# ohjay/snn-modulation-classification

Hardware: AMD Instinct MI355X
Metric: IQ windows/sec (RadioML 2x128, T=128) (higher is better)
Workload: dtype f32

## Files before the change

include/dcll_hip.h:

```cpp
#ifndef DCLL_HIP_H
#define DCLL_HIP_H

#include <stdint.h>

#ifdef __cplusplus
extern "C" {
#endif

#define DCLL_ABI_VERSION 10

enum {
    DCLL_OK = 0,
    DCLL_ERR_INVALID = -1,
    DCLL_ERR_UNSUPPORTED = -2,
    DCLL_ERR_LAUNCH = -3
};

typedef struct dcll_conv_desc {
    int32_t c_in, c_out;
    int32_t h, w;
    int32_t kh, kw;
    int32_t pad_h, pad_w;
    int32_t stride, dilation, groups;
    int32_t pool_h, pool_w;
// ... 336 lines not shown
#define DCLL_BWD_ANY     1
#define DCLL_BWD_WIDE    2
#define DCLL_BWD_SLAB    3
#define DCLL_BWD_BANDS   4
#define DCLL_BWD_POOL_DV 1u
int dcll_conv_lif_backward_ex(const dcll_conv_desc *d, const float *eps1, const float *v, const float *pv_pooled,
                              const float *g_p, const float *g_o, const float *g_pv, const float *g_v, const float *i2o_W,
                              float *dW, float *db, float *d_outW, float *d_outb, float *scratch, int64_t scratch_floats,
                              int32_t B, int32_t path, int32_t bands, uint32_t flags, void *stream);
int dcll_conv_lif_backward_ex_open(const dcll_conv_desc *d, const float *eps1, const float *v, const float *pv_pooled,
                                   const float *g_p, const float *g_o, const float *g_pv, const float *g_v, const float *i2o_W,
                                   float *d_outW, float *d_outb, float *scratch, int64_t scratch_floats, int32_t B,
                                   const float **part, int32_t *nchunk, int32_t path, int32_t bands, uint32_t flags, void *stream);
int32_t dcll_bwd_dv_pool_served(const dcll_conv_desc *d, int32_t B);

#ifdef __cplusplus
}
#endif
#endif
```

snn_modulation_classification_amd/_lib.py:

```python
import ctypes
import os
import subprocess

_PKG = os.path.dirname(os.path.abspath(__file__))
SO_PATH = os.environ.get("DCLL_HIP_SO") or os.path.join(_PKG, "libdcll_hip.so")
CSRC = os.path.join(_PKG, "csrc")

DCLL_OK, DCLL_ERR_INVALID, DCLL_ERR_UNSUPPORTED, DCLL_ERR_LAUNCH = 0, -1, -2, -3
ABI_VERSION = 10


class DCLLHipError(RuntimeError):
    pass


class DCLLUnsupported(NotImplementedError):
    pass


class ConvDesc(ctypes.Structure):
    _fields_ = [(n, ctypes.c_int32) for n in
                ("c_in", "c_out", "h", "w", "kh", "kw", "pad_h", "pad_w", "stride", "dilation", "groups",
                 "pool_h", "pool_w", "target", "output_layer", "tau_is_tensor", "refractory")] + \
               [("alpharp", ctypes.c_float), ("wrp", ctypes.c_float)]
# ... 87 lines not shown
    "dcll_grad_reduce_optim": (_I32, [ctypes.POINTER(GradParts), _I32, ctypes.POINTER(OptimTensor), _I32, _P, _P]),
    "dcll_conv_lif_backward_open_multi": (_I32, [ctypes.POINTER(BwdItem), _I32, _P]),
    "dcll_cells_to_planes": (_I32, [_P, _P, _I64, _I32, _P]),
    "dcll_dense_lif_step": (_I32, [_DDP] + [_P] * 16 + [_I32, _P]),
    "dcll_dense_lif_sequence": (_I32, [_DDP] + [_P] * 16 + [_I32, _I32, _P]),
    "dcll_dense_lif_backward": (_I32, [_DDP] + [_P] * 9 + [_I64, _I32, _P]),
    "dcll_dense_lif_backward_open": (_I32, [_DDP] + [_P] * 7 + [_I64, _I32, ctypes.POINTER(ctypes.c_void_p), _IP, _P]),
    "dcll_conv_lif_sequence": (_I32, [_DP] + [_P] * 13 + [_I32, _P, _P, _I32, _OP, _I32, _I32, _P]),
    "dcll_permute_readout": (_I32, [_P, _P, _I32, _P]),
    "dcll_conv_lif_sequence_cells": (_I32, [_DP] + [_P] * 10 + [_P, _P, _I32, _OP, _I32, _I32, _P]),
    "dcll_conv_lif_sequence_iq": (_I32, [_DP, _P, _P, _P, _P, _I32, _I32] + [_P] * 9 + [_P, _P, _I32, _OP, _I32, _I32, _P]),
    "dcll_pv_lowhigh": (_I32, [_P, _I64, _I32, _I32, _P, _P]),
    "dcll_pv_lowhigh_act": (_I32, [_P, _I64, _I32, _I32, _P, _I32, _P]),
    "dcll_readout_act_scratch": (_I64, [_I64, _I32, _I32]),
    "dcll_readout_act": (_I32, [_P] * 5 + [_I64, _I64, _I32, _I32, _I32, _P]),
    "dcll_pv_lowhigh_steps": (_I32, [_I32, _I32]),
    "dcll_readout": (_I32, [_P, _P, _P, _P, _I64, _I32, _I32, _P]),
    "dcll_readout_mode": (_I32, [_P, _P, _P, _P, _I64, _I32, _I32, _I32, _P]),
    "dcll_readout_splitk_scratch": (_I64, [_I64, _I32, _I32]),
    "dcll_readout_splitk": (_I32, [_P, _P, _P, _P, _P, _I64, _I64, _I32, _I32, _P]),
    "dcll_vote_tallies": (_I32, [_P, _I32, _P, _P, _I32, _I32, _P]),
    "dcll_step_readouts_scratch": (_I64, [_I64, _I32, _I32, _I32]),
    "dcll_step_readouts": (_I32, [_P, _P, _P, _P, _I64, _I64, _I32, _I32, _I32, _P, _P, _P, _P, _P, _P, _I32, _P]),
    "dcll_step_readouts_multi": (_I32, [ctypes.POINTER(StepRo), _I32, _P]),
    "dcll_argmax_vote": (_I32, [_P, _P, _P, _I32, _I32, _I32, _I32, _P]),
    "dcll_iq_encode": (_I32, [_P, _P, _P, _P, _P, _I32, _I32, _I32, _I32, _I32, _I32, _P]),
    "dcll_unpack_spikes": (_I32, [_P, _P, _I64, _P]),
    "dcll_pack_spikes": (_I32, [_P, _P, _I64, _P]),
    "dcll_conv_lif_sequence_any_lds": (_I64, [_DP]),
    "dcll_conv_lif_sequence_any_scratch": (_I64, [_DP]),
# ... 117 lines not shown
```

snn_modulation_classification_amd/csrc/dcll_hip.hip:

```cpp
#include "dcll_internal.h"
#include <map>
#include <mutex>
#include <utility>

static thread_local char g_err[DCLL_ERR_LEN] = "";
char *dcll_err_buf(void) { return g_err; }

extern "C" int dcll_version(void) { return DCLL_ABI_VERSION; }
extern "C" const char *dcll_last_error(void) { return g_err; }

constexpr size_t DCLL_TRACE_LEN = 1 << 16;
static thread_local bool g_trace_on = false;
static thread_local size_t g_trace_len = 0;
static thread_local char *g_trace = nullptr;
void dcll_trace_note(const char *name)
{
    if (!g_trace_on || !g_trace) return;
    const size_t n = strlen(name);
    if (g_trace_len + n + 5 >= DCLL_TRACE_LEN) {
        if (g_trace_len + 4 < DCLL_TRACE_LEN && (g_trace_len < 4 || memcmp(g_trace + g_trace_len - 4, "...\n", 4) != 0)) {
            memcpy(g_trace + g_trace_len, "...\n", 4);
            g_trace_len += 4;
        }
        return;
// ... 1883 lines not shown
                constexpr int ROW = decltype(ROWC)::value;
                const auto prs0 = tile_rsrc(pv_out + ubase), prs1 = tile_rsrc(pv_out + ubase + ustep);
                const auto vrs0 = tile_rsrc(v_out + ubase), vrs1 = tile_rsrc(v_out + ubase + ustep);
                uint32_t pk = 0;
#pragma unroll
                for (int m = 0; m < 8; ++m) {
                    const auto sw = __builtin_amdgcn_permlane16_swap(__float_as_uint(acc[2 * m]), __float_as_uint(acc[2 * m + 1]), false, false);
                    float v0 = __uint_as_float(sw[0]), v1 = __uint_as_float(sw[1]);
                    bool s0, s1;
                    if (REFRACTORY) {
                        v0 = refractory(v0, arp[m], alpharp, wrp, s0);
                        v1 = refractory(v1, arp[m], alpharp, wrp, s1);
                    } else {
                        s0 = v0 > 0.0f; s1 = v1 > 0.0f;
                    }
                    const unsigned long long mk0 = __ballot(s0), mk1 = __ballot(s1);
                    const int co = (2 * (m & 1) + 8 * (m >> 1)) * 1024 + ROW * 64;
                    if (OUT & 1) {
                        __builtin_amdgcn_raw_buffer_store_b32(__float_as_uint(sigmoidf_dev(v0)), prs0, eoff, co, 0);
                        __builtin_amdgcn_raw_buffer_store_b32(__float_as_uint(sigmoidf_dev(v1)), prs1, eoff, co, 0);
                    }
                    if (OUT & 2) {
                        __builtin_amdgcn_raw_buffer_store_b32(__float_as_uint(v0), vrs0, eoff, co, 0);
                        __builtin_amdgcn_raw_buffer_store_b32(__float_as_uint(v1), vrs1, eoff, co, 0);
                    }
                    asm("s_nop 1\n\tv_writelane_b32 %0, %1, %2" : "+v"(pk) : "s"((uint32_t)mk0), "n"(4 * m + 0));
                    asm("s_nop 1\n\tv_writelane_b32 %0, %1, %2" : "+v"(pk) : "s"((uint32_t)(mk0 >> 32)), "n"(4 * m + 1));
                    asm("s_nop 1\n\tv_writelane_b32 %0, %1, %2" : "+v"(pk) : "s"((uint32_t)mk1), "n"(4 * m + 2));
                    asm("s_nop 1\n\tv_writelane_b32 %0, %1, %2" : "+v"(pk) : "s"((uint32_t)(mk1 >> 32)), "n"(4 * m + 3));
                }
                if (spk_out && lane < 32) {
                    const auto srs = tile_rsrc(spk_out + (ubase >> 5));
                    __builtin_amdgcn_raw_buffer_store_b16((unsigned short)pk, srs, soff, 4 * (ROW >> 1) + 2 * (ROW & 1), 0);
                    __builtin_amdgcn_raw_buffer_store_b16((unsigned short)(pk >> 16), srs, soff, 32 + 4 * (ROW >> 1) + 2 * (ROW & 1), 0);
                }
            };
            epilogue(accA, arpA, std::integral_constant<int, RA>{});
            epilogue(accB, arpB, std::integral_constant<int, RB>{});

            if (!FIRST && p + 1 < NP) trace(os_write_parity(p));
            lds_barrier();
        }

        if (REFRACTORY) {
            int lo = 4 * h + rb;
            asm volatile("" : "+v"(lo));
// ... 179 lines not shown
    if (!pv || !Wt || !out || rows < 0 || K < 1 || N < 1 || (act != DCLL_ACT_NONE && act != DCLL_ACT_SIGMOID))
        return fail(DCLL_ERR_INVALID, "dcll_readout_act: bad argument");
    if (!(K % RO_KC == 0 && K < (1 << 22) && N <= 64 && (((uintptr_t)pv | (uintptr_t)Wt) & 15) == 0))
        return fail(DCLL_ERR_UNSUPPORTED, "dcll_readout_act: needs K % 32 == 0, K < 2^22, N <= 64, 16-byte aligned pv / Wt");
    hipStream_t st = (hipStream_t)stream;
    const int64_t need = dcll_readout_act_scratch(rows, K, N);
    if (need == 0) return dcll_launch_readout_t16(pv, Wt, bias, out, rows, K, N, 0, st, act);
    if (!scratch || scratch_floats < need)
        return fail(DCLL_ERR_INVALID, "dcll_readout_act: K >= 65536 is split over K and needs scratch (dcll_readout_act_scratch)");
    const int ns = act_nslice(K);
    int rc = dcll_launch_readout_t16(pv, Wt, nullptr, scratch, rows, K, N, K / ns, st, act);
    if (rc) return rc;
    hipLaunchKernelGGL(k_readout_sum, dim3(nblk(rows * N, 64)), dim3(256), 0, st, scratch, bias, out, rows * N, N, ns);
    HIP_CHECK_LAUNCH("k_readout_sum");
    return DCLL_OK;
}

constexpr int STEP_WLS = 49, STEP_WCH = 64 * STEP_WLS + 4;
__device__ __forceinline__ float buf_ldf(__amdgpu_buffer_rsrc_t rs, unsigned voff, unsigned soff)
{
    return __uint_as_float(__builtin_amdgcn_raw_buffer_load_b32(rs, voff, soff, 0));
}
__device__ __forceinline__ void buf_stf(float v, __amdgpu_buffer_rsrc_t rs, unsigned voff, unsigned soff)
{
    __builtin_amdgcn_raw_buffer_store_b32(__float_as_uint(v), rs, voff, soff, 0);
}
constexpr unsigned BUF_OOB = 0x80000000u;
template <bool Q8>
struct step_wchunk {
    static constexpr int NW = 13;
// ... 1429 lines not shown
    for (; i < per_step + stride - 1 - (per_step + stride - 1) % stride; i += stride) {
        const bool in = i < per_step;
        const float v = in ? (SIG ? sigmoidf_dev(p[i]) : p[i]) : 0.5f;
        lo += __popcll(__ballot(in && v < thr_low));
        hi += __popcll(__ballot(in && v >= thr_high));
    }
    const int lane = threadIdx.x & 63, wave = threadIdx.x >> 6;
    if (lane == 0) { red[0][wave] = lo; red[1][wave] = hi; }
    __syncthreads();
    if (threadIdx.x < 2) {
        const unsigned tot = red[threadIdx.x][0] + red[threadIdx.x][1] + red[threadIdx.x][2] + red[threadIdx.x][3];
        if (tot) atomicAdd(counts + 2 * k + threadIdx.x, (unsigned long long)tot);
    }
}

static float f32_ceil(double e)
{
    float f = (float)e;
    if ((double)f < e) f = nextafterf(f, INFINITY);
    return f;
}

static inline int n_sampled_steps(int iter0, int T) { return (iter0 + T) / 20 - iter0 / 20; }

static int launch_pv_lowhigh(const float *pv, long per_step, int T, int iter0, unsigned long long *counts,
                             hipStream_t st, const char *who, bool presig = false)
{
    if (iter0 < 0) return fail(DCLL_ERR_INVALID, "negative iteration count", who);
    const int ns = n_sampled_steps(iter0, T);
    if (ns == 0) return DCLL_OK;
    if (!pv) return fail(DCLL_ERR_INVALID, "pv statistics need the pv output of the call", who);
    if (hipMemsetAsync(counts, 0, (size_t)ns * 2 * sizeof(unsigned long long), st) != hipSuccess) {
        (void)hipGetLastError();
        return fail(DCLL_ERR_LAUNCH, "hipMemsetAsync of the pv counters failed", who);
    }
    const double e1 = 1.0 / 19.0, e18 = 18.0 * (1.0 / 19.0);
    long nb = (per_step / 4 + 255) / 256;
    if (nb < 1) nb = 1;
    if (nb > 1024) nb = 1024;
    if (presig)
        hipLaunchKernelGGL(k_pv_lowhigh<true>, dim3((unsigned)nb, (unsigned)ns), dim3(256), 0, st, pv, per_step, iter0,
                           f32_ceil(e1), f32_ceil(e18), counts);
    else
        hipLaunchKernelGGL(k_pv_lowhigh<false>, dim3((unsigned)nb, (unsigned)ns), dim3(256), 0, st, pv, per_step, iter0,
                           f32_ceil(e1), f32_ceil(e18), counts);
    HIP_CHECK_LAUNCH("k_pv_lowhigh");
    return DCLL_OK;
}

extern "C" int dcll_pv_lowhigh_act(const float *pv, int64_t per_step, int32_t T, int32_t iter0, uint64_t *counts,
                                   int32_t act, void *stream)
{
    if (T < 0 || per_step < 0 || iter0 < 0 || (act != DCLL_ACT_NONE && act != DCLL_ACT_SIGMOID))
        return fail(DCLL_ERR_INVALID, "dcll_pv_lowhigh: bad argument");
    if (T == 0 || per_step == 0 || n_sampled_steps(iter0, T) == 0) return DCLL_OK;
    if (!counts) return fail(DCLL_ERR_INVALID, "dcll_pv_lowhigh: null counters");
    return launch_pv_lowhigh(pv, per_step, T, iter0, (unsigned long long *)counts, (hipStream_t)stream, "dcll_pv_lowhigh",
                             act == DCLL_ACT_SIGMOID);
}

// ... 108 lines not shown
        if (n_ro) return fail(DCLL_ERR_UNSUPPORTED, "dcll_conv_lif_sequence: fused readout only on the 16x16 plane");
        return dcll_launch_seq_c32t(d, spk_in, W, b, tau4, eps0, eps1, arp, spk_out, pv_out, v_out, state_scratch, T, B, st);
    }
    if (n_ro == 0 && T >= DCLL_C32D_MIN_T) {
        const bool tp = (T & 1) == 0;
#define DCLL_LAUNCH_C32D(K, R, O)                                                                                       \
    hipLaunchKernelGGL((K<R, O>), dim3(B), dim3(512), 0, st, spk_in, WSRC, b, tau4, eps0, eps1, arp, spk_out, pv_out,   \
                       v_out, T, B, d->alpharp, d->wrp)
#define DCLL_LAUNCH_C32D_O(K, R)                                                                                        \
    switch (out) {                                                                                                     \
    case 0: DCLL_LAUNCH_C32D(K, R, 0); break;                                                                          \
    case 1: DCLL_LAUNCH_C32D(K, R, 1); break;                                                                          \
    case 2: DCLL_LAUNCH_C32D(K, R, 2); break;                                                                          \
    default: DCLL_LAUNCH_C32D(K, R, 3); break;                                                                         \
    }
        if (tp) {
            float *WSRC = nullptr;
            const int rc = c32d_workspace(st, &WSRC);
            if (rc) return rc;
            hipLaunchKernelGGL(k_c32d_wfrag, dim3(OS_WFRAG_FLOATS / 256), dim3(256), 0, st, W, WSRC);
            const hipError_t eh = hipGetLastError();
            if (eh != hipSuccess) {
                snprintf(dcll_err_buf(), DCLL_ERR_LEN, "k_c32d_wfrag: %s", hipGetErrorString(eh));
                return DCLL_ERR_LAUNCH;
            }
            if (d->refractory) { DCLL_LAUNCH_C32D_O(k_lif_seq_c32d, true) } else { DCLL_LAUNCH_C32D_O(k_lif_seq_c32d, false) }
            HIP_CHECK_LAUNCH("k_lif_seq_c32d");
        } else {
            const dcll_wsrc WSRC = W;
            if (d->refractory) { DCLL_LAUNCH_C32D_O(k_lif_seq_c32rp, true) } else { DCLL_LAUNCH_C32D_O(k_lif_seq_c32rp, false) }
            HIP_CHECK_LAUNCH("k_lif_seq_c32rp");
        }
#undef DCLL_LAUNCH_C32D_O
#undef DCLL_LAUNCH_C32D
        return DCLL_OK;
    }
#define DCLL_ARGS out, B, st, spk_in, W, b, tau4, eps0, eps1, arp, spk_out, pv_out, v_out, ro_Wp, ro_b, ro_out, T, d->alpharp, d->wrp
    if (d->refractory) {
        if (n_ro == 0) launch_c32<true, 0>(DCLL_ARGS);
        else if (n_ro == 24) launch_c32<true, 24>(DCLL_ARGS);
        else launch_c32<true, 48>(DCLL_ARGS);
    } else {
        if (n_ro == 0) launch_c32<false, 0>(DCLL_ARGS);
        else if (n_ro == 24) launch_c32<false, 24>(DCLL_ARGS);
        else launch_c32<false, 48>(DCLL_ARGS);
    }
#undef DCLL_ARGS
// ... 194 lines not shown
```

snn_modulation_classification_amd/csrc/dcll_internal.h:

```cpp
#pragma once
#include <hip/hip_runtime.h>
#include <type_traits>
#include <stdint.h>
#include <stdio.h>
#include <stdlib.h>
#include <string.h>

#include "../../include/dcll_hip.h"

typedef float f32x16 __attribute__((ext_vector_type(16)));
typedef float f32x4 __attribute__((ext_vector_type(4)));
typedef float f32x3 __attribute__((ext_vector_type(3)));
typedef float f32x2 __attribute__((ext_vector_type(2)));

constexpr int NWAVE = 8, CPW = 4, ROWF = 19, CHF = 361;
constexpr int IMG_FLOATS = ((32 * CHF + 3 * ROWF + 3 + 61) + 3) & ~3;
constexpr int SLOT_FLOATS = 16 * 64;

__attribute__((visibility("hidden"))) char *dcll_err_buf(void);
constexpr size_t DCLL_ERR_LEN = 512;

static inline int fail(int code, const char *msg, const char *who = nullptr)
{
    if (who) snprintf(dcll_err_buf(), DCLL_ERR_LEN, "%s: %s", who, msg);
// ... 177 lines not shown
__attribute__((visibility("hidden"))) bool dcll_dense_seq_fits(const dcll_dense_desc *d);
__attribute__((visibility("hidden")))
int dcll_launch_dense_seq(const dcll_dense_desc *d, const float *x, const float *W, const float *b, const float *alpha,
                          const float *tau_m, const float *alphas, const float *tau_s, float *eps0, float *eps1, float *arp,
                          float *out_s, float *out_pv, float *out_v, int32_t T, int32_t B, hipStream_t st);

__attribute__((visibility("hidden")))
int dcll_launch_readout_direct(const float *pv, const float *Wt, const float *bias, float *out, long rows, int K, int N,
                               hipStream_t st);

__attribute__((visibility("hidden")))
int dcll_launch_readout_t16(const float *pv, const float *Wt, const float *bias, float *out, long rows, int K, int N,
                            int kslice, hipStream_t st, int act = DCLL_ACT_NONE);

__attribute__((visibility("hidden")))
int dcll_launch_readout_t16_multi(const float *const *pv, const float *const *Wt, float *const *out, const long *rows,
                                  const int *K, const int *N, const int *kslice, int n, hipStream_t st);

__device__ __forceinline__ float sigmoidf_dev(float v) { return __builtin_amdgcn_rcpf(1.0f + __expf(-v)); }

__device__ __forceinline__ void trace_update(float x, float alpha, float tau_m, float alphas, float tau_s,
                                             float &e0, float &e1)
{
    float a = x * tau_s;
    float b = alphas * e0;
    e0 = a + b;
    float c = alpha * e1;
    float d = e0 * tau_m;
    e1 = c + d;
}
// ... 74 lines not shown
```

snn_modulation_classification_amd/csrc/dcll_readout.hip:

```cpp
#include "dcll_internal.h"

typedef __attribute__((address_space(1))) const float gfloat;
typedef __attribute__((address_space(1))) const f32x4 gf32x4;

template <int RT, int NT, int F4, int WPE>
__global__ __launch_bounds__(256) __attribute__((amdgpu_waves_per_eu(WPE, 8)))
void k_readout_direct(const float *__restrict__ pv, const float *__restrict__ Wt, const float *__restrict__ bias,
                      float *__restrict__ out, long rows, int K, int N)
{
    const int lane = threadIdx.x & 63, i = lane & 15, kq = lane >> 4;
    const int wave = __builtin_amdgcn_readfirstlane(threadIdx.x >> 6);
    const long row0 = ((long)blockIdx.x * 4 + wave) * (16 * RT);
    if (row0 >= rows) return;
    const float *abase = pv + row0 * K;
    unsigned aoff[RT], boff[NT];
#pragma unroll
    for (int rt = 0; rt < RT; ++rt) {
        long r = rt * 16 + i;
        if (row0 + r >= rows) r = rows - 1 - row0;
        aoff[rt] = (unsigned)(r * K) + 4 * F4 * kq;
    }
#pragma unroll
    for (int nt = 0; nt < NT; ++nt) {
        int n = nt * 16 + i;
// ... 58 lines not shown
}

int dcll_launch_readout_direct(const float *pv, const float *Wt, const float *bias, float *out, long rows, int K, int N,
                               hipStream_t st)
{
    const unsigned g1 = (unsigned)((rows + 63) / 64);
    if (N <= 16) hipLaunchKernelGGL((k_readout_direct<1, 1, 1, 8>), dim3(g1), dim3(256), 0, st, pv, Wt, bias, out, rows, K, N);
    else if (N <= 32) hipLaunchKernelGGL((k_readout_direct<1, 2, 1, 8>), dim3(g1), dim3(256), 0, st, pv, Wt, bias, out, rows, K, N);
    else hipLaunchKernelGGL((k_readout_direct<1, 3, 1, 8>), dim3(g1), dim3(256), 0, st, pv, Wt, bias, out, rows, K, N);
    HIP_CHECK_LAUNCH("k_readout_direct");
    return DCLL_OK;
}

constexpr int T16_ROWS = 128, T16_KC = 32, T16_LD = 36;

template <int NT, bool SIG>
__device__ __forceinline__ void readout_t16_body(const float *__restrict__ pv, const float *__restrict__ Wt,
                                                  const float *__restrict__ bias, float *__restrict__ out, const long rows,
                                                  const int K, const int N, const int kslice, const unsigned bx, const unsigned by)
{
    constexpr int NBF = (NT * 16 * 8 + 255) / 256;
    __shared__ __attribute__((aligned(16))) float sA[T16_ROWS * T16_LD];
    __shared__ __attribute__((aligned(16))) float sB[NBF * 32 * T16_LD];
    const int tid = threadIdx.x, lane = tid & 63, i = lane & 15, kq = lane >> 4;
    const int wave = __builtin_amdgcn_readfirstlane(tid >> 6);
    const long row0 = (long)bx * T16_ROWS;
    const int kc = (tid & 7) * 4, rsub = tid >> 3;
    f32x4 acc[2][NT];
#pragma unroll
    for (int rt = 0; rt < 2; ++rt)
#pragma unroll
        for (int nt = 0; nt < NT; ++nt) acc[rt][nt] = f32x4{0.f, 0.f, 0.f, 0.f};
    const long nra = rows - row0 < T16_ROWS ? rows - row0 : T16_ROWS;
    const auto ars = __builtin_amdgcn_make_buffer_rsrc((void *)(pv + row0 * K), 0, (int)(nra * K * 4), 0x00020000);
    const auto brs = __builtin_amdgcn_make_buffer_rsrc((void *)Wt, 0, (N < NT * 16 ? N : NT * 16) * K * 4, 0x00020000);
    unsigned avo[4], bvo[NBF];
#pragma unroll
    for (int q = 0; q < 4; ++q) avo[q] = 4u * (unsigned)((rsub + 32 * q) * K + kc);
#pragma unroll
    for (int q = 0; q < NBF; ++q) bvo[q] = 4u * (unsigned)((rsub + 32 * q) * K + kc);
    f32x4 ra[4], rb[NBF];
    auto fetch = [&](int k0) {
#pragma unroll
        for (int q = 0; q < 4; ++q) ra[q] = __builtin_bit_cast(f32x4, __builtin_amdgcn_raw_buffer_load_b128(ars, avo[q], 4u * k0, 2));
#pragma unroll
        for (int q = 0; q < NBF; ++q) rb[q] = __builtin_bit_cast(f32x4, __builtin_amdgcn_raw_buffer_load_b128(brs, bvo[q], 4u * k0, 0));
    };
    const int kbeg = kslice > 0 ? by * kslice : 0, kend = kslice > 0 ? kbeg + kslice : K;
    if (kslice > 0) { out += (long)by * rows * N; bias = nullptr; }
    fetch(kbeg);
    for (int k0 = kbeg; k0 < kend; k0 += T16_KC) {
#pragma unroll
        for (int q = 0; q < 4; ++q) {
            if (SIG) {
#pragma unroll
                for (int e = 0; e < 4; ++e) ra[q][e] = sigmoidf_dev(ra[q][e]);
            }
            *(f32x4 *)(sA + (rsub + 32 * q) * T16_LD + kc) = ra[q];
        }
#pragma unroll
        for (int q = 0; q < NBF; ++q) *(f32x4 *)(sB + (rsub + 32 * q) * T16_LD + kc) = rb[q];
        __syncthreads();
        if (k0 + T16_KC < kend) fetch(k0 + T16_KC);
#pragma unroll
        for (int g = 0; g < 2; ++g) {
            f32x4 a[2], b[NT];
#pragma unroll
            for (int rt = 0; rt < 2; ++rt) a[rt] = *(const f32x4 *)(sA + (wave * 32 + rt * 16 + i) * T16_LD + 16 * g + 4 * kq);
#pragma unroll
            for (int nt = 0; nt < NT; ++nt) b[nt] = *(const f32x4 *)(sB + (nt * 16 + i) * T16_LD + 16 * g + 4 * kq);
#pragma unroll
            for (int e = 0; e < 4; ++e)
#pragma unroll
                for (int rt = 0; rt < 2; ++rt)
#pragma unroll
                    for (int nt = 0; nt < NT; ++nt)
                        acc[rt][nt] = __builtin_amdgcn_mfma_f32_16x16x4f32(a[rt][e], b[nt][e], acc[rt][nt], 0, 0, 0);
        }
        __syncthreads();
    }
#pragma unroll
    for (int nt = 0; nt < NT; ++nt) {
        const int n = nt * 16 + i;
        if (n < N) {
            const float bn = bias ? bias[n] : 0.0f;
#pragma unroll
            for (int rt = 0; rt < 2; ++rt)
#pragma unroll
                for (int q = 0; q < 4; ++q) {
                    const long r = row0 + wave * 32 + rt * 16 + 4 * kq + q;
                    if (r < rows) out[r * N + n] = acc[rt][nt][q] + bn;
                }
        }
    }
}

template <int NT, bool SIG>
__global__ __launch_bounds__(256) void k_readout_t16(const float *__restrict__ pv, const float *__restrict__ Wt,
                                                      const float *__restrict__ bias, float *__restrict__ out,
                                                      long rows, int K, int N, int kslice)
{
    readout_t16_body<NT, SIG>(pv, Wt, bias, out, rows, K, N, kslice, blockIdx.x, blockIdx.y);
}
constexpr int T16M_MAX = 8;
struct readout_t16_items {
    const float *pv[T16M_MAX];
    const float *Wt[T16M_MAX];
    float *out[T16M_MAX];
    long rows[T16M_MAX];
    int K[T16M_MAX], N[T16M_MAX], kslice[T16M_MAX];
};
template <int NT>
__global__ __launch_bounds__(256) void k_readout_t16m(const readout_t16_items it)
{
    const int z = blockIdx.z;
    const long rows = it.rows[z];
    const int K = it.K[z], ks = it.kslice[z];
// ... 12 lines not shown
#define DCLL_T16(NT_)                                                                                                   \
    do {                                                                                                                \
        if (act == DCLL_ACT_SIGMOID)                                                                                    \
            hipLaunchKernelGGL((k_readout_t16<NT_, true>), g, dim3(256), 0, st, pv, Wt, bias, out, rows, K, N, kslice);  \
        else                                                                                                            \
            hipLaunchKernelGGL((k_readout_t16<NT_, false>), g, dim3(256), 0, st, pv, Wt, bias, out, rows, K, N, kslice); \
    } while (0)
    if (N <= 16) DCLL_T16(1);
    else if (N <= 32) DCLL_T16(2);
    else if (N <= 48) DCLL_T16(3);
    else DCLL_T16(4);
#undef DCLL_T16
    HIP_CHECK_LAUNCH("k_readout_t16");
    return DCLL_OK;
}
int dcll_launch_readout_t16_multi(const float *const *pv, const float *const *Wt, float *const *out, const long *rows,
                                  const int *K, const int *N, const int *kslice, int n, hipStream_t st)
{
    if (n < 1 || n > T16M_MAX) return fail(DCLL_ERR_INVALID, "readout GEMM (multi): 1 .. 8 items");
    readout_t16_items it;
    unsigned gx = 1, gy = 1;
    int nmax = 0;
    for (int i = 0; i < n; ++i) {
        if (K[i] >= (1 << 22)) return fail(DCLL_ERR_UNSUPPORTED, "readout GEMM: K above 4 M features per row");
        if (kslice[i] < 1 || K[i] % kslice[i] != 0) return fail(DCLL_ERR_INVALID, "readout GEMM (multi): split-K items only");
        it.pv[i] = pv[i], it.Wt[i] = Wt[i], it.out[i] = out[i], it.rows[i] = rows[i], it.K[i] = K[i], it.N[i] = N[i];
        it.kslice[i] = kslice[i];
        gx = max(gx, (unsigned)((rows[i] + T16_ROWS - 1) / T16_ROWS));
        gy = max(gy, (unsigned)(K[i] / kslice[i]));
        nmax = max(nmax, N[i]);
// ... 11 lines not shown
```

snn_modulation_classification_amd/networks/__init__.py:

```python
from ast import literal_eval

import os

import numpy as np
import torch
import yaml

from .. import ops, paths
from ..dcll import pytorch_libdcll as _libdcll
from ..dcll.pytorch_libdcll import Conv2dDCLLlayer, DenseDCLLlayer, DCLLClassification


def load_network_spec(yaml_path):
    with open(yaml_path, 'r') as f:
        spec = yaml.load(f, Loader=yaml.SafeLoader)
    convs = spec['conv_layers']
    for layer in convs:
        for key, val in layer.items():
            if type(val) != int:
                layer[key] = literal_eval(val)
    return convs


class ConvNetwork(torch.nn.Module):
# ... 20 lines not shown
            if learning_rates is not None:
                layer_opt['lr'] = learning_rates[min(i, len(learning_rates) - 1)]
            self.dcll_slices.append(DCLLSlice(dclllayer=layer, name='conv%d' % i, batch_size=batch_size, loss=loss,
                                              optimizer=opt, kwargs_optimizer=layer_opt, collect_stats=True,
                                              burnin=burnin))
        self._seq_buffers = {}
        self._seq_scratch = {}
        self.global_batch = None
        self.graph_learn = os.environ.get('DCLL_GRAPH_LEARN', '1') != '0'
        self._learn_graphs, self._learn_eager_steps, self._learn_last_key = {}, {}, None
        self._test_graphs, self._test_eager_steps = {}, {}
        self.graph_autotune = os.environ.get('DCLL_GRAPH_AUTOTUNE', '1') != '0'
        self._graph_tune = {}
        self.pv_budget_bytes = float(os.environ.get('DCLL_PV_BUDGET_GB', '24')) * 2 ** 30
        self.presigmoid = os.environ.get('DCLL_PRESIGMOID', 'auto')

    def learn(self, x, labels, global_batch=None):
        if global_batch is None:
            global_batch = self.global_batch
        if global_batch is not None and x.shape[0] > global_batch:
            raise ValueError('shard of %d samples of a global batch of %d: set net.global_batch (or pass global_batch=) '
                             'for THIS batch' % (x.shape[0], global_batch))
        if not all(s._native_learning() is not None for s in self.dcll_slices):
            spikes = x
            with torch.enable_grad():
                for s in self.dcll_slices:
                    spikes, _, _, _, _ = s.train_dcll(spikes, labels, regularize=False)
            return
        key = (tuple(x.shape), tuple(labels.shape))
        if key != self._learn_last_key:
# ... 528 lines not shown
            if keep_spikes:
                res['spikes'] = cat('spikes', 1)
        else:
            res = self._sequence_chunk((iq, encoder.thr_i, encoder.thr_q, int(t0), encoder.tail(B, s0, s0 + B, stot))
                                       if iq is not None else cells,
                                       'iq' if iq is not None else 'cells', T, B, dev, profile, fuse_readout,
                                       output_only=output_only, overlap=overlap_readout, keep_spikes=keep_spikes)
        if collect:
            for i, s in enumerate(self.dcll_slices):
                if res['clout'][i] is not None:
                    L = s.dclllayer
                    s.set_sequence_result(res['clout'][i], T, lowhigh=res['lowhigh'][i],
                                          numel=B * L.out_channels * int(np.prod(L.output_shape)), vote=res['vote'][i])
        return res

    def _sequence_chunk(self, first_input, first_kind, T, B, dev, profile, fuse_readout, batch_slice=None,
                        output_only=False, overlap=False, keep_spikes=False):
        for s in self.dcll_slices:
            i2h = s.dclllayer.i2h
            if batch_slice is None and (i2h.state is None or i2h.state.eps0.shape[0] != B):
                i2h.init_state(B, s.dclllayer.im_dims)
        overlap = overlap and not fuse_readout
        buf = self._sequence_buffers(T, B, dev, n_pv=self.num_layers if overlap else 1)
        main = torch.cuda.current_stream(dev)
        hot = None
        if overlap:
            if getattr(self, '_hot_stream', None) is None or self._hot_stream.device != torch.device(dev):
                self._hot_stream = torch.cuda.Stream(device=dev, priority=-1)
                self._ro_done = {}
            hot = self._hot_stream
# ... 13 lines not shown
        res = dict(logits=[], clout=[], vote=[], lowhigh=[])
        if keep_spikes:
            res['spikes'] = []
        for i, s in enumerate(self.dcll_slices):
            L = s.dclllayer
            last = (i == self.num_layers - 1)
            fused = fuse_readout and i > 0
            hidden_skip = output_only and not last
            lbuf = dict(spk=buf['spk'][i][i & 1], pv=buf['pv'][i][i if overlap else 0], ro=buf['ro'][i],
                        state_scratch=buf['state_scratch'])
            stats_iter0 = s.iter if (s.collect_stats and not hidden_skip) else None
            kind = first_kind if i == 0 else 'packed'
            Wt, bias = L.stacked_readout()
            pv_view = lbuf['pv'].reshape(T * B, -1)
            seq_ro = (not overlap and not fused and not hidden_skip and ops.readout_act_supported(pv_view, Wt))
            presig = seq_ro and (self.presigmoid == '1' or (self.presigmoid == 'auto' and L.pooling != (1, 1)))
            if overlap:
                if i in self._ro_done:
                    hot.wait_event(self._ro_done[i])
                with torch.cuda.stream(hot):
                    spk, pv, ro = timed('lif_c1' if i == 0 else 'lif_c32', L.forward_sequence, cur, T, B, kind,
                                        want_spikes=(not last) or keep_spikes, buffers=lbuf, fuse_readout=False,
                                        batch_slice=batch_slice, want_pv=not hidden_skip, lowhigh_iter0=None)
                    done = torch.cuda.Event()
                    done.record(hot)
                main.wait_event(done)
                if stats_iter0 is not None:
                    lbuf['lowhigh'] = ops.pv_lowhigh(pv.reshape(T, -1), T, stats_iter0)
            else:
                spk, pv, ro = timed('lif_c1' if i == 0 else 'lif_c32', L.forward_sequence, cur, T, B, kind,
                                    want_spikes=(not last) or keep_spikes, buffers=lbuf,
                                    fuse_readout=fused and not hidden_skip,
                                    batch_slice=batch_slice, want_pv=not hidden_skip, lowhigh_iter0=stats_iter0,
                                    presigmoid=presig)
            res['lowhigh'].append(lbuf.get('lowhigh'))
            if keep_spikes:
                res['spikes'].append(spk.clone())
            if hidden_skip:
                res['logits'].append(None)
                res['clout'].append(None)
                res['vote'].append(None)
                cur = spk
                continue
            if fused:
                p = ro[..., :self.target_size]
                logits = p
                if last:
                    logits = ro[..., self.target_size:]
                    res['o'] = logits
            else:
                pv2d = pv.reshape(T * B, -1)
                if seq_ro:
                    ro = timed('readout', ops.readout_act, pv2d, Wt, bias, out=buf['ro'][i].reshape(T * B, -1),
                               presigmoid=presig, scratch=self._seq_scratch)
                else:
                    ro = timed('readout', ops.readout, pv2d, Wt, bias, out=buf['ro'][i].reshape(T * B, -1),
                               mode=ops.READOUT_CORESIDENT if overlap else ops.READOUT_AUTO)
                if overlap:
                    self._ro_done[i] = torch.cuda.Event()
                    self._ro_done[i].record(main)
                ro = ro.reshape(T, B, -1)
                p = ro[..., :self.target_size]
                logits = p
                if last:
                    logits = ro[..., self.target_size:]
                    res['o'] = logits
            clout, vote = timed('vote', ops.argmax_vote, logits.contiguous())
# ... 139 lines not shown
```

snn_modulation_classification_amd/ops.py:

```python
import ctypes
import os
import math

import numpy as np
import torch

from . import _lib, paths
from ._lib import ACT_NONE, ACT_SIGMOID, ConvDesc, DenseDesc, IQTail, LayerOpts, check, ptr, stream_ptr


def _pair(v):
    return (int(v[0]), int(v[1])) if hasattr(v, "__len__") else (int(v), int(v))


def make_conv_desc(c_in, c_out, hw, kernel_size, padding, pooling, target, output_layer, tau_is_tensor, wrp,
                   alpharp=.65, stride=1, dilation=1, groups=1):
    (kh, kw), (pah, paw) = _pair(kernel_size), _pair(padding)
    poh, pow_ = _pair(pooling) if pooling is not None else (1, 1)
    return ConvDesc(int(c_in), int(c_out), int(hw[0]), int(hw[1]), kh, kw, pah, paw, int(stride), int(dilation),
                    int(groups), poh, pow_, int(target), int(bool(output_layer)), int(bool(tau_is_tensor)),
                    int(wrp > 0), float(alpharp), float(wrp))


def conv_lif_backward_open_multi(deferred):
# ... 685 lines not shown
        return out
    if mode != READOUT_AUTO:
        check(lib.dcll_readout_mode(ptr(pv2d), ptr(Wt), ptr(bias), ptr(out), rows, K, N, int(mode), stream_ptr()),
              "dcll_readout_mode")
        return out
    check(lib.dcll_readout(ptr(pv2d), ptr(Wt), ptr(bias), ptr(out), rows, K, N, stream_ptr()), "dcll_readout")
    return out


def readout_act_supported(pv2d, Wt):
    K, N = pv2d.shape[1], Wt.shape[0]
    return (K % 32 == 0 and (K < 65536 or K % 256 == 0) and N <= 64 and pv2d.data_ptr() % 16 == 0 and
            Wt.data_ptr() % 16 == 0 and pv2d.is_contiguous() and Wt.is_contiguous())


def readout_act(pv2d, Wt, bias, out=None, presigmoid=False, scratch=None):
    rows, K = pv2d.shape
    N = Wt.shape[0]
    if Wt.shape[1] != K:
        raise ValueError("readout: K mismatch %d vs %d" % (Wt.shape[1], K))
    _expect(pv2d, "pv", torch.float32)
    _expect(Wt, "Wt", torch.float32)
    _expect(bias, "bias", torch.float32, (N,))
    if out is None:
        out = torch.empty((rows, N), device=pv2d.device, dtype=torch.float32)
    _expect(out, "out", torch.float32, (rows, N))
    lib = _lib.get()
    need = lib.dcll_readout_act_scratch(rows, K, N)
    area = None
    if need > 0:
        area = None if scratch is None else scratch.get('act_splitk')
        if area is None or area.numel() < need:
# ... 443 lines not shown
```

Measured before the change: 22830.

## Fuse pv low/high statistics into readout GEMM and skip unused spike ballots

```diff
diff --git a/include/dcll_hip.h b/include/dcll_hip.h
--- a/include/dcll_hip.h
+++ b/include/dcll_hip.h
@@ -374,6 +374,9 @@
                                    const float **part, int32_t *nchunk, int32_t path, int32_t bands, uint32_t flags, void *stream);
 int32_t dcll_bwd_dv_pool_served(const dcll_conv_desc *d, int32_t B);
 
+int dcll_readout_act_stats(const float *pv, const float *Wt, const float *bias, float *out, int64_t rows, int32_t K, int32_t N,
+                           int32_t act, int32_t rows_per_step, int32_t iter0, uint64_t *counts, void *stream);
+
 #ifdef __cplusplus
 }
 #endif
diff --git a/snn_modulation_classification_amd/_lib.py b/snn_modulation_classification_amd/_lib.py
--- a/snn_modulation_classification_amd/_lib.py
+++ b/snn_modulation_classification_amd/_lib.py
@@ -125,6 +125,7 @@
     "dcll_pv_lowhigh_act": (_I32, [_P, _I64, _I32, _I32, _P, _I32, _P]),
     "dcll_readout_act_scratch": (_I64, [_I64, _I32, _I32]),
     "dcll_readout_act": (_I32, [_P] * 5 + [_I64, _I64, _I32, _I32, _I32, _P]),
+    "dcll_readout_act_stats": (_I32, [_P] * 4 + [_I64, _I32, _I32, _I32, _I32, _I32, _P, _P]),
     "dcll_pv_lowhigh_steps": (_I32, [_I32, _I32]),
     "dcll_readout": (_I32, [_P, _P, _P, _P, _I64, _I32, _I32, _P]),
     "dcll_readout_mode": (_I32, [_P, _P, _P, _P, _I64, _I32, _I32, _I32, _P]),
diff --git a/snn_modulation_classification_amd/csrc/dcll_hip.hip b/snn_modulation_classification_amd/csrc/dcll_hip.hip
--- a/snn_modulation_classification_amd/csrc/dcll_hip.hip
+++ b/snn_modulation_classification_amd/csrc/dcll_hip.hip
@@ -1921,7 +1921,6 @@
                     } else {
                         s0 = v0 > 0.0f; s1 = v1 > 0.0f;
                     }
-                    const unsigned long long mk0 = __ballot(s0), mk1 = __ballot(s1);
                     const int co = (2 * (m & 1) + 8 * (m >> 1)) * 1024 + ROW * 64;
                     if (OUT & 1) {
                         __builtin_amdgcn_raw_buffer_store_b32(__float_as_uint(sigmoidf_dev(v0)), prs0, eoff, co, 0);
@@ -1931,12 +1930,15 @@
                         __builtin_amdgcn_raw_buffer_store_b32(__float_as_uint(v0), vrs0, eoff, co, 0);
                         __builtin_amdgcn_raw_buffer_store_b32(__float_as_uint(v1), vrs1, eoff, co, 0);
                     }
-                    asm("s_nop 1\n\tv_writelane_b32 %0, %1, %2" : "+v"(pk) : "s"((uint32_t)mk0), "n"(4 * m + 0));
-                    asm("s_nop 1\n\tv_writelane_b32 %0, %1, %2" : "+v"(pk) : "s"((uint32_t)(mk0 >> 32)), "n"(4 * m + 1));
-                    asm("s_nop 1\n\tv_writelane_b32 %0, %1, %2" : "+v"(pk) : "s"((uint32_t)mk1), "n"(4 * m + 2));
-                    asm("s_nop 1\n\tv_writelane_b32 %0, %1, %2" : "+v"(pk) : "s"((uint32_t)(mk1 >> 32)), "n"(4 * m + 3));
+                    if constexpr ((OUT & 4) != 0) {
+                        const unsigned long long mk0 = __ballot(s0), mk1 = __ballot(s1);
+                        asm("s_nop 1\n\tv_writelane_b32 %0, %1, %2" : "+v"(pk) : "s"((uint32_t)mk0), "n"(4 * m + 0));
+                        asm("s_nop 1\n\tv_writelane_b32 %0, %1, %2" : "+v"(pk) : "s"((uint32_t)(mk0 >> 32)), "n"(4 * m + 1));
+                        asm("s_nop 1\n\tv_writelane_b32 %0, %1, %2" : "+v"(pk) : "s"((uint32_t)mk1), "n"(4 * m + 2));
+                        asm("s_nop 1\n\tv_writelane_b32 %0, %1, %2" : "+v"(pk) : "s"((uint32_t)(mk1 >> 32)), "n"(4 * m + 3));
+                    }
                 }
-                if (spk_out && lane < 32) {
+                if ((OUT & 4) && spk_out && lane < 32) {
                     const auto srs = tile_rsrc(spk_out + (ubase >> 5));
                     __builtin_amdgcn_raw_buffer_store_b16((unsigned short)pk, srs, soff, 4 * (ROW >> 1) + 2 * (ROW & 1), 0);
                     __builtin_amdgcn_raw_buffer_store_b16((unsigned short)(pk >> 16), srs, soff, 32 + 4 * (ROW >> 1) + 2 * (ROW & 1), 0);
@@ -2146,6 +2148,35 @@
     hipLaunchKernelGGL(k_readout_sum, dim3(nblk(rows * N, 64)), dim3(256), 0, st, scratch, bias, out, rows * N, N, ns);
     HIP_CHECK_LAUNCH("k_readout_sum");
     return DCLL_OK;
+}
+
+extern "C" int dcll_readout_act_stats(const float *pv, const float *Wt, const float *bias, float *out, int64_t rows,
+                                      int32_t K, int32_t N, int32_t act, int32_t rows_per_step, int32_t iter0,
+                                      uint64_t *counts, void *stream)
+{
+    const char *who = "dcll_readout_act_stats";
+    if (rows < 0 || K < 1 || N < 0 || rows_per_step < 1 || iter0 < 0 || rows % rows_per_step != 0 ||
+        rows / rows_per_step > INT32_MAX - iter0 || (act != DCLL_ACT_NONE && act != DCLL_ACT_SIGMOID))
+        return fail(DCLL_ERR_INVALID, "bad argument (rows = T x rows_per_step, iter0 >= 0, iter0 + T < 2^31)", who);
+    if (rows == 0) return DCLL_OK;
+    const int T = (int)(rows / rows_per_step);
+    const int ns = dcll_n_sampled_steps(iter0, T);
+    if (ns > 0 && !counts) return fail(DCLL_ERR_INVALID, "null counters", who);
+    if (N == 0) {
+        if (!pv) return fail(DCLL_ERR_INVALID, "bad argument", who);
+        return dcll_pv_lowhigh_act(pv, (int64_t)rows_per_step * K, T, iter0, counts, act, stream);
+    }
+    if (!pv || !Wt || !out) return fail(DCLL_ERR_INVALID, "bad argument", who);
+    if (!(K % RO_KC == 0 && K < 65536 && N <= 64 && (((uintptr_t)pv | (uintptr_t)Wt) & 15) == 0))
+        return fail(DCLL_ERR_UNSUPPORTED, "needs K % 32 == 0, K < 65536 (the unsplit readout), N <= 64, 16-byte aligned pv / Wt", who);
+    hipStream_t st = (hipStream_t)stream;
+    if (ns == 0) return dcll_launch_readout_t16(pv, Wt, bias, out, rows, K, N, 0, st, act);
+    if (hipMemsetAsync(counts, 0, (size_t)ns * 2 * sizeof(unsigned long long), st) != hipSuccess) {
+        (void)hipGetLastError();
+        return fail(DCLL_ERR_LAUNCH, "hipMemsetAsync of the pv counters failed", who);
+    }
+    return dcll_launch_readout_t16_stats(pv, Wt, bias, out, rows, K, N, st, act, rows_per_step, iter0,
+                                         (unsigned long long *)counts);
 }
 
 constexpr int STEP_WLS = 49, STEP_WCH = 64 * STEP_WLS + 4;
@@ -3605,14 +3636,7 @@
     }
 }
 
-static float f32_ceil(double e)
-{
-    float f = (float)e;
-    if ((double)f < e) f = nextafterf(f, INFINITY);
-    return f;
-}
-
-static inline int n_sampled_steps(int iter0, int T) { return (iter0 + T) / 20 - iter0 / 20; }
+static inline int n_sampled_steps(int iter0, int T) { return dcll_n_sampled_steps(iter0, T); }
 
 static int launch_pv_lowhigh(const float *pv, long per_step, int T, int iter0, unsigned long long *counts,
                              hipStream_t st, const char *who, bool presig = false)
@@ -3625,16 +3649,17 @@
         (void)hipGetLastError();
         return fail(DCLL_ERR_LAUNCH, "hipMemsetAsync of the pv counters failed", who);
     }
-    const double e1 = 1.0 / 19.0, e18 = 18.0 * (1.0 / 19.0);
+    float thr_low, thr_high;
+    dcll_pv_thresholds(&thr_low, &thr_high);
     long nb = (per_step / 4 + 255) / 256;
     if (nb < 1) nb = 1;
     if (nb > 1024) nb = 1024;
     if (presig)
         hipLaunchKernelGGL(k_pv_lowhigh<true>, dim3((unsigned)nb, (unsigned)ns), dim3(256), 0, st, pv, per_step, iter0,
-                           f32_ceil(e1), f32_ceil(e18), counts);
+                           thr_low, thr_high, counts);
     else
         hipLaunchKernelGGL(k_pv_lowhigh<false>, dim3((unsigned)nb, (unsigned)ns), dim3(256), 0, st, pv, per_step, iter0,
-                           f32_ceil(e1), f32_ceil(e18), counts);
+                           thr_low, thr_high, counts);
     HIP_CHECK_LAUNCH("k_pv_lowhigh");
     return DCLL_OK;
 }
@@ -3773,6 +3798,17 @@
     case 2: DCLL_LAUNCH_C32D(K, R, 2); break;                                                                          \
     default: DCLL_LAUNCH_C32D(K, R, 3); break;                                                                         \
     }
+#define DCLL_LAUNCH_C32D_OS(K, R)                                                                                       \
+    switch (out | (spk_out ? 4 : 0)) {                                                                                 \
+    case 0: DCLL_LAUNCH_C32D(K, R, 0); break;                                                                          \
+    case 1: DCLL_LAUNCH_C32D(K, R, 1); break;                                                                          \
+    case 2: DCLL_LAUNCH_C32D(K, R, 2); break;                                                                          \
+    case 3: DCLL_LAUNCH_C32D(K, R, 3); break;                                                                          \
+    case 4: DCLL_LAUNCH_C32D(K, R, 4); break;                                                                          \
+    case 5: DCLL_LAUNCH_C32D(K, R, 5); break;                                                                          \
+    case 6: DCLL_LAUNCH_C32D(K, R, 6); break;                                                                          \
+    default: DCLL_LAUNCH_C32D(K, R, 7); break;                                                                         \
+    }
         if (tp) {
             float *WSRC = nullptr;
             const int rc = c32d_workspace(st, &WSRC);
@@ -3783,13 +3819,14 @@
                 snprintf(dcll_err_buf(), DCLL_ERR_LEN, "k_c32d_wfrag: %s", hipGetErrorString(eh));
                 return DCLL_ERR_LAUNCH;
             }
-            if (d->refractory) { DCLL_LAUNCH_C32D_O(k_lif_seq_c32d, true) } else { DCLL_LAUNCH_C32D_O(k_lif_seq_c32d, false) }
+            if (d->refractory) { DCLL_LAUNCH_C32D_OS(k_lif_seq_c32d, true) } else { DCLL_LAUNCH_C32D_OS(k_lif_seq_c32d, false) }
             HIP_CHECK_LAUNCH("k_lif_seq_c32d");
         } else {
             const dcll_wsrc WSRC = W;
             if (d->refractory) { DCLL_LAUNCH_C32D_O(k_lif_seq_c32rp, true) } else { DCLL_LAUNCH_C32D_O(k_lif_seq_c32rp, false) }
             HIP_CHECK_LAUNCH("k_lif_seq_c32rp");
         }
+#undef DCLL_LAUNCH_C32D_OS
 #undef DCLL_LAUNCH_C32D_O
 #undef DCLL_LAUNCH_C32D
         return DCLL_OK;
diff --git a/snn_modulation_classification_amd/csrc/dcll_internal.h b/snn_modulation_classification_amd/csrc/dcll_internal.h
--- a/snn_modulation_classification_amd/csrc/dcll_internal.h
+++ b/snn_modulation_classification_amd/csrc/dcll_internal.h
@@ -1,6 +1,7 @@
 #pragma once
 #include <hip/hip_runtime.h>
 #include <type_traits>
+#include <math.h>
 #include <stdint.h>
 #include <stdio.h>
 #include <stdlib.h>
@@ -215,6 +216,23 @@
                             int kslice, hipStream_t st, int act = DCLL_ACT_NONE);
 
 __attribute__((visibility("hidden")))
+int dcll_launch_readout_t16_stats(const float *pv, const float *Wt, const float *bias, float *out, long rows, int K, int N,
+                                  hipStream_t st, int act, int rows_per_step, int iter0, unsigned long long *counts);
+
+static inline float dcll_f32_ceil(double e)
+{
+    float f = (float)e;
+    if ((double)f < e) f = nextafterf(f, INFINITY);
+    return f;
+}
+static inline void dcll_pv_thresholds(float *thr_low, float *thr_high)
+{
+    *thr_low = dcll_f32_ceil(1.0 / 19.0);
+    *thr_high = dcll_f32_ceil(18.0 * (1.0 / 19.0));
+}
+static inline int dcll_n_sampled_steps(int iter0, int T) { return (iter0 + T) / 20 - iter0 / 20; }
+
+__attribute__((visibility("hidden")))
 int dcll_launch_readout_t16_multi(const float *const *pv, const float *const *Wt, float *const *out, const long *rows,
                                   const int *K, const int *N, const int *kslice, int n, hipStream_t st);
 
diff --git a/snn_modulation_classification_amd/csrc/dcll_readout.hip b/snn_modulation_classification_amd/csrc/dcll_readout.hip
--- a/snn_modulation_classification_amd/csrc/dcll_readout.hip
+++ b/snn_modulation_classification_amd/csrc/dcll_readout.hip
@@ -96,10 +96,16 @@
 
 constexpr int T16_ROWS = 128, T16_KC = 32, T16_LD = 36;
 
-template <int NT, bool SIG>
+struct readout_stats {
+    unsigned long long *counts;
+    int B, iter0;
+    float thr_low, thr_high;
+};
+template <int NT, bool SIG, bool STATS = false>
 __device__ __forceinline__ void readout_t16_body(const float *__restrict__ pv, const float *__restrict__ Wt,
                                                   const float *__restrict__ bias, float *__restrict__ out, const long rows,
-                                                  const int K, const int N, const int kslice, const unsigned bx, const unsigned by)
+                                                  const int K, const int N, const int kslice, const unsigned bx, const unsigned by,
+                                                  const readout_stats st = readout_stats{})
 {
     constexpr int NBF = (NT * 16 * 8 + 255) / 256;
     __shared__ __attribute__((aligned(16))) float sA[T16_ROWS * T16_LD];
@@ -130,6 +136,23 @@
     };
     const int kbeg = kslice > 0 ? by * kslice : 0, kend = kslice > 0 ? kbeg + kslice : K;
     if (kslice > 0) { out += (long)by * rows * N; bias = nullptr; }
+    unsigned kfirst = 0, nk = 0, tfirst = 0, rem0 = 0;
+    if (STATS) {
+        const unsigned B = (unsigned)st.B;
+        if (row0 < (1l << 32)) { tfirst = (unsigned)row0 / B; rem0 = (unsigned)row0 % B; }
+        else { tfirst = (unsigned)(row0 / (long)B); rem0 = (unsigned)(row0 % (long)B); }
+        const unsigned tlast = tfirst + (rem0 + (unsigned)nra - 1u) / B;
+        kfirst = ((unsigned)st.iter0 + tfirst) / 20u - (unsigned)st.iter0 / 20u;
+        nk = ((unsigned)st.iter0 + tlast + 1u) / 20u - ((unsigned)st.iter0 + tfirst) / 20u;
+    }
+    auto row_iter = [&](int q) { return (unsigned)st.iter0 + tfirst + (rem0 + (unsigned)(rsub + 32 * q)) / (unsigned)st.B + 1u; };
+    unsigned lo[4] = {0, 0, 0, 0}, hi[4] = {0, 0, 0, 0};
+    bool on[4] = {false, false, false, false};
+    if (STATS && nk != 0) {
+#pragma unroll
+        for (int q = 0; q < 4; ++q) on[q] = rsub + 32 * q < nra && row_iter(q) % 20u == 0;
+    }
+    const bool count = STATS && nk != 0;
     fetch(kbeg);
     for (int k0 = kbeg; k0 < kend; k0 += T16_KC) {
 #pragma unroll
@@ -140,6 +163,15 @@
             }
             *(f32x4 *)(sA + (rsub + 32 * q) * T16_LD + kc) = ra[q];
         }
+        if (STATS && count) {
+#pragma unroll
+            for (int q = 0; q < 4; ++q)
+#pragma unroll
+                for (int e = 0; e < 4; ++e) {
+                    lo[q] += on[q] && ra[q][e] < st.thr_low;
+                    hi[q] += on[q] && ra[q][e] >= st.thr_high;
+                }
+        }
 #pragma unroll
         for (int q = 0; q < NBF; ++q) *(f32x4 *)(sB + (rsub + 32 * q) * T16_LD + kc) = rb[q];
         __syncthreads();
@@ -160,6 +192,20 @@
                         acc[rt][nt] = __builtin_amdgcn_mfma_f32_16x16x4f32(a[rt][e], b[nt][e], acc[rt][nt], 0, 0, 0);
         }
         __syncthreads();
+    }
+    if (STATS && count) {
+        for (unsigned k = kfirst; k < kfirst + nk; ++k) {
+            unsigned l = 0, h = 0;
+#pragma unroll
+            for (int q = 0; q < 4; ++q)
+                if (row_iter(q) / 20u - (unsigned)st.iter0 / 20u - 1u == k) { l += lo[q]; h += hi[q]; }
+#pragma unroll
+            for (int m = 1; m < 64; m <<= 1) { l += __shfl_xor(l, m); h += __shfl_xor(h, m); }
+            if (lane == 0) {
+                if (l) atomicAdd(st.counts + 2 * k, (unsigned long long)l);
+                if (h) atomicAdd(st.counts + 2 * k + 1, (unsigned long long)h);
+            }
+        }
     }
 #pragma unroll
     for (int nt = 0; nt < NT; ++nt) {
@@ -183,6 +229,13 @@
                                                       long rows, int K, int N, int kslice)
 {
     readout_t16_body<NT, SIG>(pv, Wt, bias, out, rows, K, N, kslice, blockIdx.x, blockIdx.y);
+}
+template <int NT, bool SIG>
+__global__ __launch_bounds__(256) void k_readout_t16_stats(const float *__restrict__ pv, const float *__restrict__ Wt,
+                                                            const float *__restrict__ bias, float *__restrict__ out,
+                                                            long rows, int K, int N, const readout_stats st)
+{
+    readout_t16_body<NT, SIG, true>(pv, Wt, bias, out, rows, K, N, 0, blockIdx.x, 0, st);
 }
 constexpr int T16M_MAX = 8;
 struct readout_t16_items {
@@ -225,6 +278,29 @@
     HIP_CHECK_LAUNCH("k_readout_t16");
     return DCLL_OK;
 }
+int dcll_launch_readout_t16_stats(const float *pv, const float *Wt, const float *bias, float *out, long rows, int K, int N,
+                                  hipStream_t st, int act, int rows_per_step, int iter0, unsigned long long *counts)
+{
+    if (K >= (1 << 22)) return fail(DCLL_ERR_UNSUPPORTED, "readout GEMM: K above 4 M features per row");
+    readout_stats rs;
+    rs.counts = counts, rs.B = rows_per_step, rs.iter0 = iter0;
+    dcll_pv_thresholds(&rs.thr_low, &rs.thr_high);
+    const dim3 g((unsigned)((rows + T16_ROWS - 1) / T16_ROWS));
+#define DCLL_T16S(NT_)                                                                                                  \
+    do {                                                                                                                \
+        if (act == DCLL_ACT_SIGMOID)                                                                                    \
+            hipLaunchKernelGGL((k_readout_t16_stats<NT_, true>), g, dim3(256), 0, st, pv, Wt, bias, out, rows, K, N, rs);  \
+        else                                                                                                            \
+            hipLaunchKernelGGL((k_readout_t16_stats<NT_, false>), g, dim3(256), 0, st, pv, Wt, bias, out, rows, K, N, rs); \
+    } while (0)
+    if (N <= 16) DCLL_T16S(1);
+    else if (N <= 32) DCLL_T16S(2);
+    else if (N <= 48) DCLL_T16S(3);
+    else DCLL_T16S(4);
+#undef DCLL_T16S
+    HIP_CHECK_LAUNCH("k_readout_t16_stats");
+    return DCLL_OK;
+}
 int dcll_launch_readout_t16_multi(const float *const *pv, const float *const *Wt, float *const *out, const long *rows,
                                   const int *K, const int *N, const int *kslice, int n, hipStream_t st)
 {
diff --git a/snn_modulation_classification_amd/networks/__init__.py b/snn_modulation_classification_amd/networks/__init__.py
--- a/snn_modulation_classification_amd/networks/__init__.py
+++ b/snn_modulation_classification_amd/networks/__init__.py
@@ -58,6 +58,7 @@
         self._graph_tune = {}
         self.pv_budget_bytes = float(os.environ.get('DCLL_PV_BUDGET_GB', '24')) * 2 ** 30
         self.presigmoid = os.environ.get('DCLL_PRESIGMOID', 'auto')
+        self.readout_stats = os.environ.get('DCLL_READOUT_STATS', '0') != '0'
 
     def learn(self, x, labels, global_batch=None):
         if global_batch is None:
@@ -616,6 +617,16 @@
                                           numel=B * L.out_channels * int(np.prod(L.output_shape)), vote=res['vote'][i])
         return res
 
+    PRESIGMOID_AUTO = ()
+
+    def _presigmoid_layer(self, i, L):
+        if self.presigmoid in ('0', '1'):
+            return self.presigmoid == '1'
+        if L.pooling != (1, 1):
+            return True
+        pos = 'first' if i == 0 else ('last' if i == self.num_layers - 1 else 'middle')
+        return pos in (self.PRESIGMOID_AUTO if self.presigmoid == 'auto' else self.presigmoid.split(','))
+
     def _sequence_chunk(self, first_input, first_kind, T, B, dev, profile, fuse_readout, batch_slice=None,
                         output_only=False, overlap=False, keep_spikes=False):
         for s in self.dcll_slices:
@@ -659,7 +670,9 @@
             Wt, bias = L.stacked_readout()
             pv_view = lbuf['pv'].reshape(T * B, -1)
             seq_ro = (not overlap and not fused and not hidden_skip and ops.readout_act_supported(pv_view, Wt))
-            presig = seq_ro and (self.presigmoid == '1' or (self.presigmoid == 'auto' and L.pooling != (1, 1)))
+            presig = seq_ro and self._presigmoid_layer(i, L)
+            ro_stats = (seq_ro and stats_iter0 is not None and self.readout_stats and
+                        ops.readout_act_stats_supported(pv_view, Wt))
             if overlap:
                 if i in self._ro_done:
                     hot.wait_event(self._ro_done[i])
@@ -676,8 +689,8 @@
                 spk, pv, ro = timed('lif_c1' if i == 0 else 'lif_c32', L.forward_sequence, cur, T, B, kind,
                                     want_spikes=(not last) or keep_spikes, buffers=lbuf,
                                     fuse_readout=fused and not hidden_skip,
-                                    batch_slice=batch_slice, want_pv=not hidden_skip, lowhigh_iter0=stats_iter0,
-                                    presigmoid=presig)
+                                    batch_slice=batch_slice, want_pv=not hidden_skip,
+                                    lowhigh_iter0=None if ro_stats else stats_iter0, presigmoid=presig)
             res['lowhigh'].append(lbuf.get('lowhigh'))
             if keep_spikes:
                 res['spikes'].append(spk.clone())
@@ -695,7 +708,11 @@
                     res['o'] = logits
             else:
                 pv2d = pv.reshape(T * B, -1)
-                if seq_ro:
+                if ro_stats:
+                    ro, lbuf['lowhigh'] = timed('readout', ops.readout_act, pv2d, Wt, bias,
+                                                out=buf['ro'][i].reshape(T * B, -1), presigmoid=presig, stats=(B, stats_iter0))
+                    res['lowhigh'][-1] = lbuf['lowhigh']
+                elif seq_ro:
                     ro = timed('readout', ops.readout_act, pv2d, Wt, bias, out=buf['ro'][i].reshape(T * B, -1),
                                presigmoid=presig, scratch=self._seq_scratch)
                 else:
diff --git a/snn_modulation_classification_amd/ops.py b/snn_modulation_classification_amd/ops.py
--- a/snn_modulation_classification_amd/ops.py
+++ b/snn_modulation_classification_amd/ops.py
@@ -723,8 +723,31 @@
             Wt.data_ptr() % 16 == 0 and pv2d.is_contiguous() and Wt.is_contiguous())
 
 
-def readout_act(pv2d, Wt, bias, out=None, presigmoid=False, scratch=None):
+def readout_act_stats_supported(pv2d, Wt):
+    return readout_act_supported(pv2d, Wt) and pv2d.shape[1] < 65536
+
+
+def readout_act(pv2d, Wt, bias, out=None, presigmoid=False, scratch=None, stats=None):
     rows, K = pv2d.shape
+    if stats is not None:
+        rows_per_step, iter0 = int(stats[0]), int(stats[1])
+        N = Wt.shape[0]
+        if Wt.shape[1] != K:
+            raise ValueError("readout: K mismatch %d vs %d" % (Wt.shape[1], K))
+        if rows_per_step < 1 or rows % rows_per_step:
+            raise ValueError("readout statistics: %d rows are not whole steps of %d rows" % (rows, rows_per_step))
+        _expect(pv2d, "pv", torch.float32)
+        _expect(Wt, "Wt", torch.float32)
+        _expect(bias, "bias", torch.float32, (N,))
+        if out is None:
+            out = torch.empty((rows, N), device=pv2d.device, dtype=torch.float32)
+        _expect(out, "out", torch.float32, (rows, N))
+        counts = torch.empty((pv_lowhigh_steps(iter0, rows // rows_per_step), 2), device=pv2d.device, dtype=torch.int64)
+        check(_lib.get().dcll_readout_act_stats(ptr(pv2d), ptr(Wt), ptr(bias), ptr(out), rows, K, N,
+                                                ACT_SIGMOID if presigmoid else ACT_NONE, rows_per_step, iter0,
+                                                ptr(counts) if counts.numel() else None, stream_ptr()),
+              "dcll_readout_act_stats")
+        return out, counts
     N = Wt.shape[0]
     if Wt.shape[1] != K:
         raise ValueError("readout: K mismatch %d vs %d" % (Wt.shape[1], K))
```

Result: no change. 22890 (median of 6 runs) (+0.3%).
